# Quyans/GOI-Hyperplane

Hardware: AMD Instinct MI355X
Metric: training views/sec (rasterizer fwd+bwd), 1M Gaussians @1600x1056 RGB+16-d feat (higher is better)
Workload: dtype f32

## Files before the change

goi_hyperplane_amd/csrc/render_bwd.hip:

```cpp
#include "blend_common.h"

namespace goi {

namespace {


#if !defined(GOI_BWD_WAVES)
#define GOI_BWD_WAVES 4
#endif
#define GOI_BWD_LAUNCH_BOUNDS __launch_bounds__(64, (S4 <= 4 ? GOI_BWD_WAVES : 2))

#ifndef GOI_TSTRIDE
#define GOI_TSTRIDE 66
#endif
constexpr int GROUP = 8;
constexpr int BATCH = 32;
constexpr int TSTRIDE = GOI_TSTRIDE;

template <int S4>
struct BwdCfg {
    static constexpr int NF4 = 1 + S4;
    static constexpr int NSEM = 4 * S4;
    static constexpr int NCH = NSEM + 4;
    static constexpr int NB = (NSEM + 15) / 16;
};

template <int S4, bool F16, bool MASKS>
__global__ GOI_BWD_LAUNCH_BOUNDS void render_bwd_rows_k(
    const uint2* __restrict__ ranges, const uint32_t* __restrict__ point_list, int W, int H, int gx, int gy,
    int n_quads, int S, const GaussRec* __restrict__ rec, const float* __restrict__ semantics,
    const int* __restrict__ radii, const uint4* __restrict__ aux, const float* __restrict__ bg,
    const float* __restrict__ out_alpha, const uint32_t* __restrict__ n_contrib, const float* __restrict__ dL_dpix,
    const float* __restrict__ dL_dpixsem, const float* __restrict__ dL_dpixdepth, const float* __restrict__ dL_dalphas,
    float* __restrict__ rows, uint8_t* __restrict__ flags, int row_floats,
    const uint32_t* __restrict__ counters, const uint32_t* __restrict__ qorder,
    const unsigned long long* __restrict__ qmask0, const unsigned long long* __restrict__ qmask,
    const uint32_t* __restrict__ qcost) {
    using Cfg = BwdCfg<S4>;
    const bool cull = counters[COUNTER_CULL] != 0;
    constexpr int NF4 = Cfg::NF4, NSEM = Cfg::NSEM, NCH = Cfg::NCH, NB = Cfg::NB;
    __shared__ f32x4 s_geo[BATCH + GROUP];
    __shared__ f32x4 s_geo2[BATCH + GROUP];
    __shared__ float2 s_cen[BATCH + GROUP];
    __shared__ __attribute__((aligned(16))) float4 s_feat[BATCH * NF4];
    constexpr int TS = TSTRIDE;
    constexpr int T_BYTES = F16 ? F16_FLOATS * 4 : 2 * GROUP * TSTRIDE * 4;
    __shared__ __attribute__((aligned(16))) char s_traw[T_BYTES];
    float* const s_t = reinterpret_cast<float*>(s_traw);

    const QuadGeom t = quad_geom_of(qorder ? (int)qorder[quad_slot()] : quad_slot(), W, H, gx, n_quads);
    if (t.tile < 0) return;
    if (counters[COUNTER_OVF]) return;
    const int lane = t.lane;
    const uint2 range = ranges[t.tile];
    const size_t HW = (size_t)W * H;
    const size_t pix_id = (size_t)W * t.py + t.px;
    const size_t pix_ld = t.inside ? pix_id : 0;
    const uint32_t nc_ld = n_contrib[pix_ld];
    const float oa_ld = out_alpha[pix_ld];
    float dLch[NCH];
    if (dL_dpixsem && S == NSEM) {
#pragma unroll
        for (int ch = 0; ch < NSEM; ch++) dLch[ch] = dL_dpixsem[ch * HW + pix_ld];
    } else {
#pragma unroll
        for (int ch = 0; ch < NSEM; ch++) dLch[ch] = (dL_dpixsem && ch < S) ? dL_dpixsem[ch * HW + pix_ld] : 0.f;
    }
    dLch[NSEM + 0] = dL_dpix ? dL_dpix[0 * HW + pix_ld] : 0.f;
    dLch[NSEM + 1] = dL_dpix ? dL_dpix[1 * HW + pix_ld] : 0.f;
    dLch[NSEM + 2] = dL_dpix ? dL_dpix[2 * HW + pix_ld] : 0.f;
    dLch[NSEM + 3] = dL_dpixdepth ? dL_dpixdepth[pix_ld] : 0.f;
    float dLa = dL_dalphas ? dL_dalphas[pix_ld] : 0.f;

    const int last_contributor = t.inside ? (int)nc_ld : 0;
    const int n_proc = qcost ? (int)qcost[__builtin_amdgcn_readfirstlane(4 * t.tile + t.q)] : wave_max_i32(last_contributor);
    if (n_proc == 0) return;
    const int rounds = (n_proc + BATCH - 1) / BATCH;

    const float T_final = t.inside ? (1.f - oa_ld) : 0.f;
    float T = T_final;
    if (!t.inside) {
#pragma unroll
        for (int ch = 0; ch < NCH; ch++) dLch[ch] = 0.f;
        dLa = 0.f;
    }
    const float bg_dot = bg[0] * dLch[NSEM] + bg[1] * dLch[NSEM + 1] + bg[2] * dLch[NSEM + 2];
    float R = 0.f;
    f32x2 dL2[NCH / 2];
#pragma unroll
    for (int i = 0; i < NCH / 2; i++) dL2[i] = f32x2{dLch[2 * i], dLch[2 * i + 1]};
    const f32x4* s_feat4 = reinterpret_cast<const f32x4*>(s_feat);

    const int kq = lane >> 4, mm = lane & 15;
    float bfrag[F16 ? 1 : NB][F16 ? 1 : 16];
    float bmix[F16 ? 1 : 16];
    f16x8 Wh[F16 ? NB : 1][2], Wl[F16 ? NB : 1][2], Cc[2];
    float unscale[F16 ? NB : 1], unscale_c = 0.f;
    bf16x8 Bas;
    constexpr int BT = 17;
    static_assert(64 * BT * 4 <= F16_FLOATS * 4 && 64 * 16 * 4 <= T_BYTES, "staging region too small");
    const float k1 = mm == 4 ? 1.f : 0.f, ku = mm == 5 ? 1.f : 0.f, kv = mm == 6 ? 1.f : 0.f;
    const float kuu = mm == 7 ? 1.f : 0.f, kuv = mm == 8 ? 1.f : 0.f, kvv = mm == 9 ? 1.f : 0.f;
    auto basis = [&](int p) {
        const float u = (float)(p & 7) - 3.5f, v = (float)(p >> 3) - 3.5f;
        return k1 + ku * u + kv * v + kuu * (u * u) + kuv * (u * v) + kvv * (v * v);
    };
    if constexpr (F16) {
#pragma unroll
        for (int nb = 0; nb < NB; nb++) {
#pragma unroll
            for (int c = 0; c < 16; c++) {
                const int ch = nb * 16 + c;
                s_t[lane * BT + c] = ch < NSEM ? dLch[ch] : 0.f;
            }
            __builtin_amdgcn_wave_barrier();
            float y[2][8];
#pragma unroll
            for (int c2 = 0; c2 < 2; c2++)
#pragma unroll
                for (int i = 0; i < 8; i++) y[c2][i] = s_t[(32 * c2 + 8 * kq + i) * BT + mm];
            f16_b_operand(y, Wh[nb], Wl[nb], unscale[nb]);
            __builtin_amdgcn_wave_barrier();
        }
        {
#pragma unroll
            for (int c = 0; c < 4; c++) s_t[lane * 5 + c] = dLch[NSEM + c];
            __builtin_amdgcn_wave_barrier();
            float y[2][8];
#pragma unroll
            for (int c2 = 0; c2 < 2; c2++)
#pragma unroll
                for (int i = 0; i < 8; i++) y[c2][i] = s_t[(32 * c2 + 8 * kq + i) * 5 + (mm & 3)];
            f16x8 hi[2], lo[2];
            f16_b_operand(y, hi, lo, unscale_c);
            typedef uint32_t u32x4 __attribute__((ext_vector_type(4)));
#pragma unroll
            for (int c2 = 0; c2 < 2; c2++) {
                const u32x4 hu = __builtin_bit_cast(u32x4, hi[c2]), lu = __builtin_bit_cast(u32x4, lo[c2]);
                u32x4 cu;
#pragma unroll
                for (int i = 0; i < 4; i++) cu[i] = mm < 4 ? hu[i] : mm < 8 ? lu[i] : 0u;
                Cc[c2] = __builtin_bit_cast(f16x8, cu);
            }
            __builtin_amdgcn_wave_barrier();
        }
        {
            float y[8];
            const float vb = (float)kq - 1.5f;
#pragma unroll
            for (int i = 0; i < 8; i++) {
                const float u = (float)i - 3.5f;
                y[i] = mm == 0 ? 1.f : mm == 1 ? u : mm == 2 ? vb : mm == 3 ? u * u : mm == 4 ? u * vb : mm == 5 ? vb * vb : 0.f;
            }
            bf16x8 unused;
            split_pack8(y, Bas, unused);
        }
    } else {
#pragma unroll
        for (int nb = 0; nb < NB; nb++) {
#pragma unroll
            for (int c = 0; c < 16; c++) {
                const int ch = nb * 16 + c;
                s_t[lane * 16 + c] = ch < NSEM ? dLch[ch] : 0.f;
            }
            __builtin_amdgcn_wave_barrier();
#pragma unroll
            for (int s = 0; s < 16; s++) bfrag[nb][s] = s_t[(4 * s + kq) * 16 + mm];
            __builtin_amdgcn_wave_barrier();
        }
#pragma unroll
        for (int c = 0; c < 4; c++) s_t[lane * 4 + c] = dLch[NSEM + c];
        __builtin_amdgcn_wave_barrier();
#pragma unroll
        for (int s = 0; s < 16; s++) bmix[s] = mm < 4 ? s_t[(4 * s + kq) * 4 + mm] : basis(4 * s + kq);
        __builtin_amdgcn_wave_barrier();
    }
    auto uniform = [](float x) { return __int_as_float(__builtin_amdgcn_readfirstlane(__float_as_int(x))); };
    const float QCX = uniform(t.QX0 + 3.5f), QCY = uniform(t.QY0 + 3.5f);
    const f32x2 uv = {t.pxf - QCX, t.pyf - QCY};
    const float half_W = uniform(0.5f * W), half_H = uniform(0.5f * H);

    uint32_t id_n = 0;
    unsigned long long w_n = 0;
    float4 q0_n = make_float4(0, 0, 0, 0), q1_n = make_float4(1.f, 0.f, -1.f, -1.f);
    const int tile_u = __builtin_amdgcn_readfirstlane(t.tile), q_u = __builtin_amdgcn_readfirstlane(t.q);
    const uint32_t x0_u = (uint32_t)__builtin_amdgcn_readfirstlane((int)range.x);
    auto prefetch = [&](int b) {
        if constexpr (MASKS) {
            w_n = *member_mask_ptr(const_cast<unsigned long long*>(qmask0), const_cast<unsigned long long*>(qmask), tile_u, q_u,
                                   x0_u, b >> 1);
            const int pos = b * BATCH + lane;
            if (lane < BATCH && pos < n_proc) id_n = point_list[range.x + (uint32_t)pos];
        } else {
            const int k = b * BATCH + lane;
            q1_n.z = -1.f;
            if (lane < BATCH && k < n_proc) {
                id_n = point_list[range.x + (n_proc - 1 - k)];
                const float4* r4 = reinterpret_cast<const float4*>(rec + id_n);
                q0_n = r4[0];
                q1_n = r4[1];
            }
        }
    };
    prefetch(MASKS ? rounds - 1 : 0);

    int nslot = 0;
    unsigned long long jpack = 0;

    auto xrow = [](int rho) { return rho * 8 + 16 * (rho >> 3); };
    auto flush_group = [&](int cnt) {
        f32x4 acc[NB];
        f32x4 accx = {0.f, 0.f, 0.f, 0.f};
#pragma unroll
        for (int nb = 0; nb < NB; nb++) acc[nb] = f32x4{0.f, 0.f, 0.f, 0.f};
        __builtin_amdgcn_wave_barrier();
        if constexpr (F16) {
            const f32x4* wsrc = reinterpret_cast<const f32x4*>(s_t + f16_lane_offset(mm, kq));
            {
                const f32x4* src = wsrc + (f16_row(GROUP) - f16_row(0)) / 4;
                const f32x4 a0 = src[0], a1 = src[1];
                const float y[8] = {a0.x, a0.y, a0.z, a0.w, a1.x, a1.y, a1.z, a1.w};
                bf16x8 Hh, Hl, Ht;
                split3_pack8(y, Hh, Hl, Ht);
                accx = __builtin_amdgcn_mfma_f32_16x16x32_bf16(Ht, Bas, accx, 0, 0, 0);
                accx = __builtin_amdgcn_mfma_f32_16x16x32_bf16(Hl, Bas, accx, 0, 0, 0);
                accx = __builtin_amdgcn_mfma_f32_16x16x32_bf16(Hh, Bas, accx, 0, 0, 0);
            }
            f32x4 accc = {0.f, 0.f, 0.f, 0.f};
            {
                f16x8 A0, A1;
                f16_a_operands(wsrc, A0, A1);
#pragma unroll
                for (int nb = 0; nb < NB; nb++) {
                    acc[nb] = __builtin_amdgcn_mfma_f32_16x16x32_f16(A0, Wl[nb][0], acc[nb], 0, 0, 0);
                    acc[nb] = __builtin_amdgcn_mfma_f32_16x16x32_f16(A1, Wl[nb][1], acc[nb], 0, 0, 0);
                    acc[nb] = __builtin_amdgcn_mfma_f32_16x16x32_f16(A0, Wh[nb][0], acc[nb], 0, 0, 0);
                    acc[nb] = __builtin_amdgcn_mfma_f32_16x16x32_f16(A1, Wh[nb][1], acc[nb], 0, 0, 0);
                }
                accc = __builtin_amdgcn_mfma_f32_16x16x32_f16(A0, Cc[0], accc, 0, 0, 0);
                accc = __builtin_amdgcn_mfma_f32_16x16x32_f16(A1, Cc[1], accc, 0, 0, 0);
            }
            __builtin_amdgcn_wave_barrier();
            if (mm < 8) {
                float* xb = s_t + xrow(4 * kq) + mm;
#pragma unroll
                for (int r = 0; r < 4; r++) xb[8 * r] = accx[r];
            }
            f32x2 sem[NB];
#pragma unroll
            for (int nb = 0; nb < NB; nb++) sem[nb] = (acc[nb].xy + acc[nb].zw) * unscale[nb];
            f32x2 col = accc.xy + accc.zw;
            col.x += __int_as_float(__builtin_amdgcn_update_dpp(0, __float_as_int(col.x), 0x104, 0xF, 0xF, true));
            col.y += __int_as_float(__builtin_amdgcn_update_dpp(0, __float_as_int(col.y), 0x104, 0xF, 0xF, true));
            col *= unscale_c;
#pragma unroll
            for (int e = 0; e < 2; e++) {
                const int j = 2 * kq + e;
                if (j < cnt) {
                    const int idx = (int)((jpack >> (8 * j)) & 0xFF);
                    float* dst = rows + (size_t)__float_as_uint(s_geo2[idx].w) * row_floats;
#pragma unroll
                    for (int nb = 0; nb < NB; nb++) {
                        const int ch = nb * 16 + mm;
                        if (ch < NSEM) dst[ch] = sem[nb][e];
                    }
                    if (mm < 4) dst[NSEM + mm] = col[e];
                }
            }
        } else {
#pragma unroll
            for (int s = 0; s < 16; s++) {
                const float a = s_t[mm * TS + 4 * s + kq];
#pragma unroll
                for (int nb = 0; nb < NB; nb++)
                    acc[nb] = __builtin_amdgcn_mfma_f32_16x16x4f32(a, bfrag[nb][s], acc[nb], 0, 0, 0);
                accx = __builtin_amdgcn_mfma_f32_16x16x4f32(a, bmix[s], accx, 0, 0, 0);
            }
        }
        __builtin_amdgcn_wave_barrier();
#pragma unroll
        for (int r = 0; r < 4 && !F16; r++) {
            const int row = 4 * kq + r;
            if (row >= GROUP && mm >= 4 && mm < 12) s_t[(row - GROUP) * 8 + (mm - 4)] = accx[r];
            if (row < cnt) {
                const int idx = (int)((jpack >> (8 * row)) & 0xFF);
                float* dst = rows + (size_t)__float_as_uint(s_geo2[idx].w) * row_floats;
#pragma unroll
                for (int nb = 0; nb < NB; nb++) {
                    const int ch = nb * 16 + mm;
                    if (ch < NSEM) dst[ch] = acc[nb][r];
                }
                if (mm < 4) dst[NSEM + mm] = accx[r];
            }
        }
        __builtin_amdgcn_wave_barrier();
        if (lane < cnt) {
            const float4 m03 = *reinterpret_cast<const float4*>(&s_t[lane * 8]);
            const float2 m45 = *reinterpret_cast<const float2*>(&s_t[lane * 8 + 4]);
            const int idx = (int)((jpack >> (8 * lane)) & 0xFF);
            const f32x4 g = s_geo[idx];
            const f32x4 g2 = s_geo2[idx];
            const float2 cen = s_cen[idx];
            const uint32_t slot = __float_as_uint(g2.w);
            const float Dx = cen.x, Dy = cen.y;
            float ca, cb, cc, inv_o;
            coef_decode(g, g2, ca, cb, cc, inv_o);
            float m0, sx, sy, sxx, sxy, syy;
            auto shift = [&](const float4& a, const float2& b, float DX, float DY) {
                m0 += a.x;
                sx += DX * a.x - a.y;
                sy += DY * a.x - a.z;
                sxx += DX * DX * a.x - 2.f * DX * a.y + a.w;
                sxy += DX * DY * a.x - DX * a.z - DY * a.y + b.x;
                syy += DY * DY * a.x - 2.f * DY * a.z + b.y;
            };
            m0 = sx = sy = sxx = sxy = syy = 0.f;
            if constexpr (F16) {
                const int r1 = 4 * (lane >> 1) + (lane & 1);
                shift(*reinterpret_cast<const float4*>(&s_t[xrow(r1)]), *reinterpret_cast<const float2*>(&s_t[xrow(r1) + 4]), Dx, Dy + 2.f);
                shift(*reinterpret_cast<const float4*>(&s_t[xrow(r1 + 2)]), *reinterpret_cast<const float2*>(&s_t[xrow(r1 + 2) + 4]), Dx, Dy - 2.f);
            } else {
                shift(m03, m45, Dx, Dy);
            }
            float* dst = rows + (size_t)slot * row_floats + NCH;
            dst[0] = -half_W * (ca * sx + cb * sy);
            dst[1] = -half_H * (cc * sy + cb * sx);
            dst[2] = -0.5f * sxx;
            dst[3] = -0.5f * sxy;
            dst[4] = -0.5f * syy;
            dst[5] = m0 * inv_o;
            flags[slot] = 1;
        }
        __builtin_amdgcn_wave_barrier();
    };

    for (int bi = 0; bi < rounds; bi++) {
        const int b = MASKS ? rounds - 1 - bi : bi;
        const uint32_t id = id_n;
        float4 q0 = q0_n, q1 = q1_n;
        bool hit;
        unsigned long long m;
        if constexpr (MASKS) {
            const uint32_t mem = (uint32_t)__builtin_amdgcn_readfirstlane((int)(uint32_t)(w_n >> (32 * (b & 1))));
            m = mem;
            hit = lane < BATCH && ((mem >> lane) & 1u);
            if (bi + 1 < rounds) prefetch(b - 1);
        } else {
            hit = ellipse_hits_quadrant(q0.x, q0.y, q0.z, q0.w, q1.x, q1.y, q1.z, q1.w, t.QX0, t.QY0);
            if (bi + 1 < rounds) prefetch(b + 1);
            m = __ballot(hit);
        }
        if (m == 0) continue;
        if (hit) {
            const float4* r4 = reinterpret_cast<const float4*>(rec + id);
            const float* srow = semantics + (size_t)id * S;
            const bool rows_of_float4 = (S & 3) == 0;
            lds_dma16(r4 + 2, &s_feat[0]);
            if (rows_of_float4) {
#pragma unroll
                for (int i = 0; i < S4; i++)
                    lds_dma16(reinterpret_cast<const float4*>(srow) + i, &s_feat[(1 + i) * BATCH]);
            }
            if constexpr (MASKS) {
                q0 = r4[0];
                q1 = r4[1];
            }
            int x0, y0, x1, y1;
            const uint4 ax = aux[id];
            listed_rect(q0.x, q0.y, (int)ax.y, q1.z, q1.w, cull, gx, gy, x0, y0, x1, y1);
            const uint32_t inst = ax.x + tile_instance(aux_mask(ax), t.tx, t.ty, x0, y0, x1);
            const PolyCoef pc = poly_coefs(q0.x, q0.y, q0.z, q0.w, q1.x, q1.y, QCX, QCY);
            int sl = lane;
            asm volatile("" : "+v"(sl));
            s_geo[sl] = f32x4{pc.A35.x, pc.A35.y, pc.A12.x, pc.A12.y};
            s_geo2[sl] = f32x4{pc.A0, pc.A4, pc.lim, __uint_as_float(inst * 4u + (uint32_t)t.q)};
            s_cen[sl] = make_float2(q0.x - QCX, q0.y - QCY);
            if (!rows_of_float4) {
#pragma unroll
                for (int i = 0; i < S4; i++) {
                    float4 v;
                    v.x = (4 * i + 0 < S) ? srow[4 * i + 0] : 0.f;
                    v.y = (4 * i + 1 < S) ? srow[4 * i + 1] : 0.f;
                    v.z = (4 * i + 2 < S) ? srow[4 * i + 2] : 0.f;
                    v.w = (4 * i + 3 < S) ? srow[4 * i + 3] : 0.f;
                    s_feat[(1 + i) * BATCH + sl] = v;
                }
            }
        }
        __builtin_amdgcn_s_waitcnt(0x0F70);
        __builtin_amdgcn_wave_barrier();

        while (m) {
            int j, pos0;
            if constexpr (MASKS) {
                j = 31 - __builtin_clz((uint32_t)m);
                m &= ~(1ull << j);
                pos0 = b * BATCH + j;
            } else {
                j = __builtin_ctzll(m);
                m &= m - 1;
                pos0 = n_proc - 1 - (b * BATCH + j);
            }
            const f32x4 g = s_geo[j];
            const f32x4 g2 = s_geo2[j];
            const PairEval e = eval_poly(g.xy, g.zw, g2.x, g2.y, g2.z, uv);
            const bool live = pos0 < last_contributor;
            if constexpr (!MASKS)
                if (!any_all(live, e.below, e.seen)) continue;
            const bool c = live && e.hit;

            const f32x4 f0 = s_feat4[j];
            f32x2 da = f0.xy * dL2[NSEM / 2];
            f32x2 db = f0.zw * dL2[NSEM / 2 + 1];
#pragma unroll
            for (int i = 0; i < S4; i++) {
                const f32x4 f = s_feat4[(1 + i) * BATCH + j];
                da = __builtin_elementwise_fma(f.xy, dL2[2 * i], da);
                db = __builtin_elementwise_fma(f.zw, dL2[2 * i + 1], db);
            }
            const f32x2 dot2 = da + db;
            const float dotv = (dot2.x + dot2.y) + dLa;
            const float one_m_a = 1.f - e.alpha;
            const float inv = __builtin_amdgcn_rcpf(one_m_a);
            const float Tn = T * inv;
            float wgt = 0.f, hval = 0.f;
            if (c) {
                const float dL_dopa = (dotv - R) * Tn - (T_final * inv) * bg_dot;
                R = e.alpha * dotv + one_m_a * R;
                T = Tn;
                wgt = e.alpha * Tn;
                hval = e.E * dL_dopa;
            }
            if constexpr (F16) {
                const int wrow = nslot * 72 + ((nslot & 1) << 2);
                s_t[wrow + lane] = wgt;
                s_t[wrow + lane + (f16_row(GROUP) - f16_row(0))] = hval;
            } else {
                s_t[nslot * TS + lane] = wgt;
                s_t[(GROUP + nslot) * TS + lane] = hval;
            }
            jpack |= (unsigned long long)j << (8 * nslot);
            nslot++;
            if (nslot == GROUP) {
                flush_group(GROUP);
                nslot = 0;
                jpack = 0;
            }
        }
        __builtin_amdgcn_wave_barrier();
        if (nslot > 0 && bi + 1 < rounds) {
            const int idx = (int)((jpack >> (8 * (lane & 7))) & 0xFF);
            if (lane < nslot) {
                s_geo[BATCH + lane] = s_geo[idx];
                s_geo2[BATCH + lane] = s_geo2[idx];
                s_cen[BATCH + lane] = s_cen[idx];
            }
            constexpr unsigned long long CARRY = 0x0706050403020100ull + 0x0101010101010101ull * BATCH;
            jpack = CARRY & ((1ull << (8 * nslot)) - 1ull);
            __builtin_amdgcn_wave_barrier();
        }
    }
    if (nslot > 0) flush_group(nslot);
}

constexpr int QO_THREADS = 1024, QO_WAVES = QO_THREADS / 64, QO_BUCKETS = 64, QO_ROUNDS = 16;
constexpr int QO_CLEAR_BLOCKS = 248;
__global__ __launch_bounds__(QO_THREADS) void quad_order_k(const uint32_t* __restrict__ qcost, int n_quads, int per,
                                                           uint32_t* __restrict__ qorder, int shift,
                                                           uint8_t* __restrict__ clear_flags,
                                                           const uint32_t* __restrict__ n_dev, uint32_t cap,
                                                           uint32_t* __restrict__ clear_ctl) {
    if (blockIdx.x >= 8) {
        if (clear_ctl && blockIdx.x == 8 && threadIdx.x < 8) clear_ctl[threadIdx.x] = 0u;
        if (!clear_flags) return;
        const size_t nq = ((size_t)min(*n_dev, cap) * 4 + 15) / 16;
        uint4* dst = reinterpret_cast<uint4*>(clear_flags);
        for (size_t i = (size_t)(blockIdx.x - 8) * QO_THREADS + threadIdx.x; i < nq; i += (size_t)QO_CLEAR_BLOCKS * QO_THREADS)
            dst[i] = make_uint4(0u, 0u, 0u, 0u);
        return;
    }
    __shared__ uint32_t cnt[QO_WAVES][QO_BUCKETS];
    const int band = blockIdx.x, base = band * per;
    const int n = max(0, min(per, n_quads - base));
    const int lane = threadIdx.x & 63, w = threadIdx.x >> 6;
    for (int i = threadIdx.x; i < QO_WAVES * QO_BUCKETS; i += QO_THREADS) (&cnt[0][0])[i] = 0;
    __syncthreads();
    const int chunk = (per + QO_WAVES - 1) / QO_WAVES;
    const unsigned long long lt = (1ull << lane) - 1ull;
    uint32_t d_r[QO_ROUNDS], rank_r[QO_ROUNDS];
#pragma unroll
    for (int r = 0; r < QO_ROUNDS; r++) {
        if (r * 64 >= chunk) break;
        const int e = w * chunk + r * 64 + lane;
        const bool ok = r * 64 + lane < chunk && e < n;
        const uint32_t c = ok ? qcost[base + e] : 0u;
        const uint32_t d = (uint32_t)(QO_BUCKETS - 1) - min((uint32_t)(QO_BUCKETS - 1), c >> shift);
        unsigned long long peers = __ballot(ok);
#pragma unroll
        for (int b = 0; b < 6; b++) {
            const bool bit = (d >> b) & 1u;
            const unsigned long long bal = __ballot(bit);
            peers &= bit ? bal : ~bal;
        }
        const uint32_t prev = ok ? cnt[w][d] : 0u;
        const uint32_t below = (uint32_t)__popcll(peers & lt);
        d_r[r] = d;
        rank_r[r] = prev + below;
        __builtin_amdgcn_wave_barrier();
        if (ok && below == 0) cnt[w][d] = prev + (uint32_t)__popcll(peers);
        __builtin_amdgcn_wave_barrier();
    }
    __syncthreads();
    if (threadIdx.x < 64) {
        uint32_t tot = 0;
        for (int ww = 0; ww < QO_WAVES; ww++) tot += cnt[ww][lane];
        uint32_t incl = tot;
#pragma unroll
        for (int dd = 1; dd < 64; dd <<= 1) {
            const uint32_t o = __shfl_up(incl, dd, 64);
            if (lane >= dd) incl += o;
        }
        uint32_t run = incl - tot;
        for (int ww = 0; ww < QO_WAVES; ww++) {
            const uint32_t t = cnt[ww][lane];
            cnt[ww][lane] = run;
            run += t;
        }
    }
    __syncthreads();
#pragma unroll
    for (int r = 0; r < QO_ROUNDS; r++) {
        const int e = w * chunk + r * 64 + lane;
        if (r * 64 + lane < chunk && e < n) qorder[base + cnt[w][d_r[r]] + rank_r[r]] = (uint32_t)(base + e);
    }
    for (int i = n + threadIdx.x; i < per; i += QO_THREADS) qorder[base + i] = 0xFFFFFFFFu;
}

template <int S4>
void launch_bwd_rows_s4(const GoiRasterScene& sc, const GeomView& g, const ImageView& im, const uint32_t* point_list,
                        const int* radii, const float* out_alpha, const PixelGrads& dpix, const BwdScratchView& scr,
                        bool exact_flush, bool walk_masks, hipStream_t s, const unsigned long long* qmask) {
    const int gx = (sc.W + TILE - 1) / TILE, gy = (sc.H + TILE - 1) / TILE;
    const int n_quads = gx * gy * 4;
#define GOI_LAUNCH_ROWS(F16, MASKS)                                                                                    \
    render_bwd_rows_k<S4, F16, MASKS><<<dim3(quad_grid(n_quads)), dim3(64), 0, s>>>(                                     \
        im.ranges, point_list, sc.W, sc.H, gx, gy, n_quads, sc.S, g.rec, sc.semantics, radii, g.aux, sc.bg, out_alpha, \
        im.n_contrib, dpix.color, dpix.semantic, dpix.depth, dpix.alpha, scr.rows, scr.flags, bwd_row_floats(sc.S),    \
        g.counters, quad_order_enabled(sc.W, sc.H) ? im.qorder : nullptr, im.qmask0, qmask, im.qcost)
    const bool masks = qmask != nullptr && walk_masks;
    if (exact_flush) {
        if (masks) GOI_LAUNCH_ROWS(false, true);
        else GOI_LAUNCH_ROWS(false, false);
    } else {
        if (masks) GOI_LAUNCH_ROWS(true, true);
        else GOI_LAUNCH_ROWS(true, false);
    }
#undef GOI_LAUNCH_ROWS
}

}

bool quad_order_enabled(int W, int H) {
    const int gx = (W + TILE - 1) / TILE, gy = (H + TILE - 1) / TILE;
    const int per = quad_grid(gx * gy * 4) / 8;
    return g_options.bwd_order != 0 && (per + QO_WAVES - 1) / QO_WAVES <= 64 * QO_ROUNDS;
}

bool launch_quad_order(const GoiRasterScene& sc, const ImageView& im, hipStream_t s, uint8_t* clear_flags,
                       const uint32_t* n_dev, uint32_t cap, uint32_t* clear_ctl) {
    if (!quad_order_enabled(sc.W, sc.H)) return false;
    const int gx = (sc.W + TILE - 1) / TILE, gy = (sc.H + TILE - 1) / TILE;
    const int n_quads = gx * gy * 4, per = quad_grid(n_quads) / 8;
    quad_order_k<<<dim3(clear_flags ? 8 + QO_CLEAR_BLOCKS : 8), dim3(QO_THREADS), 0, s>>>(
        im.qcost, n_quads, per, im.qorder, 3 + g_options.bwd_order, clear_flags, n_dev, cap, clear_ctl);
    return true;
}

void launch_render_bwd_rows(const GoiRasterScene& sc, const GeomView& g, const ImageView& im, const uint32_t* point_list,
                            const int* radii, const float* out_alpha, const PixelGrads& dpix, const BwdScratchView& scr,
                            bool exact_flush, bool walk_masks, hipStream_t s, const unsigned long long* qmask) {
#define GOI_CALL(N) launch_bwd_rows_s4<N>(sc, g, im, point_list, radii, out_alpha, dpix, scr, exact_flush, walk_masks, s, qmask)
    GOI_DISPATCH_S4(sc.S, GOI_CALL)
#undef GOI_CALL
}

}
```

Measured before the change: 806.6.

## Defer moment expansion to process two flushed groups per wave pass

New measurement: 815.0 (median of 6 runs). About the same (+1.0%).

```diff
diff --git a/goi_hyperplane_amd/csrc/render_bwd.hip b/goi_hyperplane_amd/csrc/render_bwd.hip
--- a/goi_hyperplane_amd/csrc/render_bwd.hip
+++ b/goi_hyperplane_amd/csrc/render_bwd.hip
@@ -39,13 +39,16 @@
     using Cfg = BwdCfg<S4>;
     const bool cull = counters[COUNTER_CULL] != 0;
     constexpr int NF4 = Cfg::NF4, NSEM = Cfg::NSEM, NCH = Cfg::NCH, NB = Cfg::NB;
-    __shared__ f32x4 s_geo[BATCH + GROUP];
-    __shared__ f32x4 s_geo2[BATCH + GROUP];
-    __shared__ float2 s_cen[BATCH + GROUP];
+    constexpr int PARK = BATCH + GROUP;
+    __shared__ f32x4 s_geo[PARK + GROUP];
+    __shared__ f32x4 s_geo2[PARK + GROUP];
+    __shared__ float2 s_cen[PARK + GROUP];
     __shared__ __attribute__((aligned(16))) float4 s_feat[BATCH * NF4];
     constexpr int TS = TSTRIDE;
     constexpr int T_BYTES = F16 ? F16_FLOATS * 4 : 2 * GROUP * TSTRIDE * 4;
-    __shared__ __attribute__((aligned(16))) char s_traw[T_BYTES];
+    constexpr int XPARK = T_BYTES / 4, XROWS_FLOATS = 2 * GROUP * 8 + 16;
+    static_assert(T_BYTES % 16 == 0, "the parking area is read as float4");
+    __shared__ __attribute__((aligned(16))) char s_traw[T_BYTES + XROWS_FLOATS * 4];
     float* const s_t = reinterpret_cast<float*>(s_traw);
 
     const QuadGeom t = quad_geom_of(qorder ? (int)qorder[quad_slot()] : quad_slot(), W, H, gx, n_quads);
@@ -206,9 +209,10 @@
 
     int nslot = 0;
     unsigned long long jpack = 0;
+    unsigned long long ppack = 0;
 
     auto xrow = [](int rho) { return rho * 8 + 16 * (rho >> 3); };
-    auto flush_group = [&](int cnt) {
+    auto flush_products = [&](int cnt, int xoff) {
         f32x4 acc[NB];
         f32x4 accx = {0.f, 0.f, 0.f, 0.f};
 #pragma unroll
@@ -242,7 +246,7 @@
             }
             __builtin_amdgcn_wave_barrier();
             if (mm < 8) {
-                float* xb = s_t + xrow(4 * kq) + mm;
+                float* xb = s_t + xoff + xrow(4 * kq) + mm;
 #pragma unroll
                 for (int r = 0; r < 4; r++) xb[8 * r] = accx[r];
             }
@@ -281,7 +285,7 @@
 #pragma unroll
         for (int r = 0; r < 4 && !F16; r++) {
             const int row = 4 * kq + r;
-            if (row >= GROUP && mm >= 4 && mm < 12) s_t[(row - GROUP) * 8 + (mm - 4)] = accx[r];
+            if (row >= GROUP && mm >= 4 && mm < 12) s_t[xoff + (row - GROUP) * 8 + (mm - 4)] = accx[r];
             if (row < cnt) {
                 const int idx = (int)((jpack >> (8 * row)) & 0xFF);
                 float* dst = rows + (size_t)__float_as_uint(s_geo2[idx].w) * row_floats;
@@ -294,10 +298,15 @@
             }
         }
         __builtin_amdgcn_wave_barrier();
-        if (lane < cnt) {
-            const float4 m03 = *reinterpret_cast<const float4*>(&s_t[lane * 8]);
-            const float2 m45 = *reinterpret_cast<const float2*>(&s_t[lane * 8 + 4]);
-            const int idx = (int)((jpack >> (8 * lane)) & 0xFF);
+    };
+    auto expand_moments = [&](int n_lo, int n_hi) {
+        const bool cur = lane >= GROUP;
+        if (lane < (cur ? GROUP + n_hi : n_lo)) {
+            const int l = lane & (GROUP - 1);
+            const float* const xt = s_t + (cur ? 0 : XPARK);
+            const float4 m03 = *reinterpret_cast<const float4*>(&xt[l * 8]);
+            const float2 m45 = *reinterpret_cast<const float2*>(&xt[l * 8 + 4]);
+            const int idx = (int)(((cur ? jpack : ppack) >> (8 * l)) & 0xFF);
             const f32x4 g = s_geo[idx];
             const f32x4 g2 = s_geo2[idx];
             const float2 cen = s_cen[idx];
@@ -316,9 +325,9 @@
             };
             m0 = sx = sy = sxx = sxy = syy = 0.f;
             if constexpr (F16) {
-                const int r1 = 4 * (lane >> 1) + (lane & 1);
-                shift(*reinterpret_cast<const float4*>(&s_t[xrow(r1)]), *reinterpret_cast<const float2*>(&s_t[xrow(r1) + 4]), Dx, Dy + 2.f);
-                shift(*reinterpret_cast<const float4*>(&s_t[xrow(r1 + 2)]), *reinterpret_cast<const float2*>(&s_t[xrow(r1 + 2) + 4]), Dx, Dy - 2.f);
+                const int r1 = 4 * (l >> 1) + (l & 1);
+                shift(*reinterpret_cast<const float4*>(&xt[xrow(r1)]), *reinterpret_cast<const float2*>(&xt[xrow(r1) + 4]), Dx, Dy + 2.f);
+                shift(*reinterpret_cast<const float4*>(&xt[xrow(r1 + 2)]), *reinterpret_cast<const float2*>(&xt[xrow(r1 + 2) + 4]), Dx, Dy - 2.f);
             } else {
                 shift(m03, m45, Dx, Dy);
             }
@@ -332,6 +341,15 @@
             flags[slot] = 1;
         }
         __builtin_amdgcn_wave_barrier();
+    };
+    auto flush_group = [&]() {
+        flush_products(GROUP, ppack ? 0 : XPARK);
+        if (ppack) {
+            expand_moments(GROUP, GROUP);
+            ppack = 0;
+        } else {
+            ppack = jpack;
+        }
     };
 
     for (int bi = 0; bi < rounds; bi++) {
@@ -442,12 +460,22 @@
             jpack |= (unsigned long long)j << (8 * nslot);
             nslot++;
             if (nslot == GROUP) {
-                flush_group(GROUP);
+                flush_group();
                 nslot = 0;
                 jpack = 0;
             }
         }
         __builtin_amdgcn_wave_barrier();
+        if (ppack && bi + 1 < rounds) {
+            const int idx = (int)((ppack >> (8 * (lane & 7))) & 0xFF);
+            if (lane < GROUP) {
+                s_geo[PARK + lane] = s_geo[idx];
+                s_geo2[PARK + lane] = s_geo2[idx];
+                s_cen[PARK + lane] = s_cen[idx];
+            }
+            ppack = 0x0706050403020100ull + 0x0101010101010101ull * PARK;
+            __builtin_amdgcn_wave_barrier();
+        }
         if (nslot > 0 && bi + 1 < rounds) {
             const int idx = (int)((jpack >> (8 * (lane & 7))) & 0xFF);
             if (lane < nslot) {
@@ -460,7 +488,12 @@
             __builtin_amdgcn_wave_barrier();
         }
     }
-    if (nslot > 0) flush_group(nslot);
+    const bool parked = ppack != 0;
+    if (nslot > 0) {
+        flush_products(nslot, parked ? 0 : XPARK);
+        if (!parked) ppack = jpack;
+    }
+    if (parked || nslot > 0) expand_moments(parked ? GROUP : nslot, parked ? nslot : 0);
 }
 
 constexpr int QO_THREADS = 1024, QO_WAVES = QO_THREADS / 64, QO_BUCKETS = 64, QO_ROUNDS = 16;
```
